# massquantity/tdfo

Hardware: AMD Instinct MI355X
Metric: examples/sec (whole node) DLRM on Criteo-1TB-shaped synthetic (higher is better)
Workload: dtype bf16; 1 GPU; model=DLRM, global_batch=8192, parallelism=single-gpu, tables=criteo-1tb, embedding_dim=128, per_gpu_batch=8192

## Files before the change

csrc/bindings.cpp:

```cpp
#include <cmath>
#include <cstring>

#include <ATen/ATen.h>
#include <ATen/hip/HIPContext.h>
#include <torch/library.h>

#include "tdfo_kernels.h"

namespace {

using at::Tensor;

hipStream_t cur_stream() { return at::hip::getCurrentHIPStream().stream(); }

const uint16_t* bf16_ptr(const Tensor& t) {
  TORCH_CHECK(t.scalar_type() == at::kBFloat16, "expected bf16 tensor");
  return reinterpret_cast<const uint16_t*>(t.data_ptr());
}
uint16_t* bf16_mut(const Tensor& t) {
  TORCH_CHECK(t.scalar_type() == at::kBFloat16, "expected bf16 tensor");
  return reinterpret_cast<uint16_t*>(t.data_ptr());
}
void check_dev(const Tensor& t, const char* name) {
  TORCH_CHECK(t.is_cuda(), name, " must be a GPU tensor");
}
void check_2d_rowmajor(const Tensor& t, const char* name) {
  TORCH_CHECK(t.dim() == 2, name, " must be 2-D");
  TORCH_CHECK(t.stride(1) == 1, name, " must have unit inner stride");
}
bool aligned16(const void* p) { return (reinterpret_cast<uintptr_t>(p) & 15) == 0; }

struct GemmBatch {
  bool on = false;
  std::vector<tdfo::GemmArgs> args;
  std::vector<Tensor> keep;
};
thread_local GemmBatch g_gemm_batch;

void gemm_batch_begin() {
  TORCH_CHECK(!g_gemm_batch.on, "gemm_batch: already open");
  g_gemm_batch.on = true;
}

void gemm_batch_end() {
  GemmBatch& b = g_gemm_batch;
  b.on = false;
  if (!b.args.empty()) tdfo::gemm_group(b.args.data(), (int)b.args.size(), cur_stream());
  b.args.clear();
  b.keep.clear();
}

void gemm(const Tensor& a_in, bool a_col, const Tensor& b_in, bool b_col,
          const c10::optional<Tensor>& bias, bool relu,
          const c10::optional<Tensor>& mask, const c10::optional<Tensor>& out,
          const c10::optional<Tensor>& out32, int64_t splits, const c10::optional<Tensor>& mul,
          const c10::optional<Tensor>& add, const c10::optional<Tensor>& out2, int64_t ldc32,
          int64_t csum_col) {
  check_dev(a_in, "a"); check_dev(b_in, "b");
  check_2d_rowmajor(a_in, "a"); check_2d_rowmajor(b_in, "b");
  const int64_t Ka = a_col ? a_in.size(0) : a_in.size(1);
  const int64_t Kb = b_col ? b_in.size(0) : b_in.size(1);
  TORCH_CHECK(Ka == Kb && Ka > 0, "gemm: K mismatch ", Ka, " vs ", Kb);
  Tensor a = a_in, b = b_in;
  if (Ka % 64) {
    const int64_t Kp = (Ka + 63) / 64 * 64;
    auto pad = [&](const Tensor& t, bool col) {
      Tensor z = col ? at::zeros({Kp, t.size(1)}, t.options()) : at::zeros({t.size(0), Kp}, t.options());
      if (col) z.narrow(0, 0, Ka).copy_(t); else z.narrow(1, 0, Ka).copy_(t);
      return z;
    };
    a = pad(a_in, a_col);
    b = pad(b_in, b_col);
  }
  const int64_t M = a_col ? a.size(1) : a.size(0);
  const int64_t K = a_col ? a.size(0) : a.size(1);
  const int64_t N = b_col ? b.size(1) : b.size(0);
  TORCH_CHECK(M > 0 && N > 0, "gemm: empty output");
  TORCH_CHECK(a.stride(0) % 8 == 0 && b.stride(0) % 8 == 0, "gemm: ld must be multiple of 8");
  TORCH_CHECK(aligned16(a.data_ptr()) && aligned16(b.data_ptr()), "gemm: operands must be 16-B aligned");
  if (a_col) TORCH_CHECK(M % 8 == 0 && M >= 8, "gemm: col-layout A needs M % 8 == 0");
  if (b_col) TORCH_CHECK(N % 8 == 0 && N >= 8, "gemm: col-layout B needs N % 8 == 0");
  TORCH_CHECK(splits >= 1 && splits <= K / 64, "gemm: bad split count");
  TORCH_CHECK(splits == 1 || !(bias || relu || mask),
              "gemm: splits > 1 takes no bias, relu or mask (the epilogue would act on every "
              "partial sum)");
  tdfo::GemmArgs g{};
  g.A = bf16_ptr(a); g.lda = a.stride(0); g.a_col = a_col;
  g.B = bf16_ptr(b); g.ldb = b.stride(0); g.b_col = b_col;
  g.M = (int)M; g.N = (int)N; g.K = (int)K; g.splits = (int)splits;
  if (bias) {
    check_dev(*bias, "bias");
    TORCH_CHECK(bias->scalar_type() == at::kFloat && bias->dim() == 1 && bias->numel() == N,
                "gemm: bias must be fp32 [N] (any stride)");
    g.bias = bias->data_ptr<float>(); g.bias_stride = bias->stride(0);
  }
  g.relu = relu;
  if (mask) {
    check_2d_rowmajor(*mask, "mask");
    TORCH_CHECK(mask->size(0) == M && mask->size(1) == N, "gemm: mask shape");
    g.mask = bf16_ptr(*mask); g.ldm = mask->stride(0);
  }
  TORCH_CHECK(out || out32 || out2, "gemm: need an output");
  if (out) {
    check_2d_rowmajor(*out, "out");
    TORCH_CHECK(out->size(0) == M && out->size(1) == N, "gemm: out shape");
    g.C = bf16_mut(*out); g.ldc = out->stride(0);
    TORCH_CHECK(splits == 1, "gemm: bf16 output requires splits == 1");
  }
  if (out32) {
    TORCH_CHECK(out32->scalar_type() == at::kFloat && out32->is_contiguous(), "gemm: out32 fp32 contiguous");
    const int64_t ld32 = ldc32 > 0 ? ldc32 : N;
    TORCH_CHECK(ld32 >= N && ld32 % 4 == 0, "gemm: ldc32 must be >= N and a multiple of 4");
    TORCH_CHECK(out32->numel() >= splits * M * ld32, "gemm: out32 too small");
    g.C32 = out32->data_ptr<float>(); g.ldc32 = ld32;
    if (csum_col >= 0) {
      TORCH_CHECK(a_col && csum_col >= N && csum_col < ld32,
                  "gemm: csum_col needs a col-layout A and N <= csum_col < ldc32");
      g.csum_on = 1; g.csum_col = (int)csum_col;
    }
  }
  TORCH_CHECK(csum_col < 0 || out32, "gemm: csum_col needs out32");
  auto check_mn = [&](const c10::optional<Tensor>& t, const char* name) {
    check_2d_rowmajor(*t, name);
    TORCH_CHECK(t->size(0) == M && t->size(1) == N && t->stride(0) % 8 == 0 &&
                aligned16(t->data_ptr()), "gemm: ", name, " must be [M, N], 16-B aligned rows");
  };
  if (mul) { check_mn(mul, "mul"); g.mul = bf16_ptr(*mul); g.ldmul = mul->stride(0); }
  if (add) { check_mn(add, "add"); g.add = bf16_ptr(*add); g.ldadd = add->stride(0); }
  if (out2) {
    check_mn(out2, "out2");
    TORCH_CHECK(splits == 1, "gemm: out2 requires splits == 1");
    g.C2 = bf16_mut(*out2); g.ldc2 = out2->stride(0);
  }
  TORCH_CHECK(!(mul || add) || out2, "gemm: mul/add need out2");
  if (g_gemm_batch.on) {
    g_gemm_batch.args.push_back(g);
    g_gemm_batch.keep.push_back(a);
    g_gemm_batch.keep.push_back(b);
    return;
  }
  tdfo::gemm_bf16(g, cur_stream());
}

tdfo::SlotMap make_slots(at::IntArrayRef off, at::IntArrayRef stride, int64_t F) {
  TORCH_CHECK((int64_t)off.size() >= F && (int64_t)stride.size() >= F, "slot map too short");
  tdfo::SlotMap m{};
  for (int64_t i = 0; i < F && i < 32; ++i) { m.off[i] = off[i]; m.stride[i] = stride[i]; }
  return m;
}

void check_inter(int64_t F, int64_t D) {
  TORCH_CHECK(F >= 2 && F <= 32, "interaction: F must be in [2, 32]");
  TORCH_CHECK(D == 16 || D == 32 || D == 64 || D == 128 || D == 256,
              "interaction: D must be 16/32/64/128/256");
}

void check_slots_fit(const Tensor& emb, const tdfo::SlotMap& m, int64_t F, int64_t D, int64_t B) {
  for (int64_t i = 1; i < F; ++i) {
    TORCH_CHECK(m.off[i] % 8 == 0 && m.stride[i] % 8 == 0, "slot offsets must be multiples of 8");
    TORCH_CHECK(m.off[i] >= 0 && m.off[i] + (B - 1) * m.stride[i] + D <= emb.numel(),
                "interaction: slot ", i, " out of range");
  }
}

void interaction_fwd(const Tensor& dense, const Tensor& emb, at::IntArrayRef off,
                     at::IntArrayRef stride, int64_t F, int64_t D, const Tensor& out,
                     int64_t ones_col) {
  check_dev(dense, "dense"); check_dev(emb, "emb"); check_dev(out, "out");
  check_inter(F, D); check_2d_rowmajor(dense, "dense"); check_2d_rowmajor(out, "out");
  const int64_t B = dense.size(0);
  TORCH_CHECK(dense.size(1) >= D && dense.stride(0) % 8 == 0, "dense shape");
  TORCH_CHECK(out.size(0) == B && out.size(1) >= D + F * (F - 1) / 2 && out.size(1) % 8 == 0 &&
              out.stride(0) == out.size(1), "interaction out must be [B, ldo] contiguous, ldo%8==0");
  TORCH_CHECK(emb.is_contiguous() && aligned16(emb.data_ptr()) && aligned16(dense.data_ptr()) &&
              aligned16(out.data_ptr()), "alignment");
  auto m = make_slots(off, stride, F);
  check_slots_fit(emb, m, F, D, B);
  tdfo::interaction_fwd(bf16_ptr(dense), dense.stride(0), bf16_ptr(emb), m, (int)F, (int)D,
                        (int)B, bf16_mut(out), out.stride(0), (int)ones_col, cur_stream());
}

void interaction_bwd(const Tensor& dz, const Tensor& dense, const Tensor& emb,
                     at::IntArrayRef off, at::IntArrayRef stride, int64_t F, int64_t D,
                     const Tensor& d_dense, const Tensor& d_emb, at::IntArrayRef doff,
                     at::IntArrayRef dstride, bool relu_mask) {
  check_dev(dz, "dz"); check_dev(dense, "dense"); check_dev(emb, "emb");
  check_dev(d_dense, "d_dense"); check_dev(d_emb, "d_emb");
  check_inter(F, D);
  check_2d_rowmajor(dz, "dz"); check_2d_rowmajor(dense, "dense"); check_2d_rowmajor(d_dense, "d_dense");
  const int64_t B = dense.size(0);
  TORCH_CHECK(dz.size(0) == B && dz.size(1) >= D + F * (F - 1) / 2, "dz shape");
  TORCH_CHECK(d_dense.size(0) == B && d_dense.size(1) >= D, "d_dense shape");
  TORCH_CHECK(dz.stride(0) % 8 == 0 && aligned16(dz.data_ptr()), "dz alignment");
  TORCH_CHECK(d_dense.stride(0) % 8 == 0 && aligned16(d_dense.data_ptr()) &&
              aligned16(d_emb.data_ptr()), "d_dense / d_emb alignment (16-B row stores)");
  TORCH_CHECK(emb.is_contiguous() && d_emb.is_contiguous(), "emb contiguous");
  auto m = make_slots(off, stride, F);
  auto dm = make_slots(doff, dstride, F);
  check_slots_fit(emb, m, F, D, B);
  check_slots_fit(d_emb, dm, F, D, B);
  tdfo::interaction_bwd(bf16_ptr(dz), dz.stride(0), bf16_ptr(dense), dense.stride(0),
                        bf16_ptr(emb), m, (int)F, (int)D, (int)B, bf16_mut(d_dense),
                        d_dense.stride(0), bf16_mut(d_emb), dm, relu_mask, cur_stream());
}

tdfo::AttnArgs attn_args(const Tensor& qkv, const Tensor& ids, int64_t H, double rate,
                         int64_t seed, const c10::optional<Tensor>& step, int64_t pad_id,
                         bool stream = false) {
  check_dev(qkv, "qkv"); check_dev(ids, "ids");
  TORCH_CHECK(qkv.scalar_type() == at::kFloat && qkv.is_contiguous() && qkv.dim() == 3,
              "attention: qkv fp32 contiguous [B, T, 3E]");
  TORCH_CHECK(ids.scalar_type() == at::kLong && ids.is_contiguous() && ids.dim() == 2 &&
              ids.size(0) == qkv.size(0) && ids.size(1) == qkv.size(1), "attention: ids int64 [B, T]");
  const int64_t E3 = qkv.size(2);
  TORCH_CHECK(E3 % 3 == 0 && H > 0 && (E3 / 3) % H == 0, "attention: 3E must split into H heads");
  if (stream) {
    TORCH_CHECK(qkv.size(1) > tdfo::ATTN_SHORT_MAXT && qkv.size(1) <= tdfo::ATTN_STREAM_MAXT,
                "attention (streaming): 64 < T <= 4096");
  } else {
    TORCH_CHECK(qkv.size(1) <= tdfo::ATTN_LONG_MAXT,
                "attention: T <= 512 (one-wave kernel up to 64, tiled kernel with lse above)");
  }
  TORCH_CHECK(rate >= 0.0 && rate < 1.0, "attention: dropout rate in [0, 1)");
  tdfo::AttnArgs a{};
  a.qkv = qkv.data_ptr<float>(); a.ids = ids.data_ptr<int64_t>();
  a.B = (int)qkv.size(0); a.T = (int)qkv.size(1); a.H = (int)H; a.dk = (int)(E3 / 3 / H);
  a.scale = 1.f / std::sqrt((float)a.dk); a.rate = (float)rate; a.seed = seed; a.pad_id = pad_id;
  if (step) {
    check_dev(*step, "step");
    TORCH_CHECK(step->scalar_type() == at::kLong && step->numel() >= 1, "attention: step int64");
    a.step = step->data_ptr<int64_t>();
  }
  return a;
}

// ... 1970 lines not shown
```

csrc/include/tdfo_kernels.h:

```cpp
#pragma once
#include <hip/hip_runtime.h>
#include <stdint.h>

namespace tdfo {

struct GemmArgs {
  const uint16_t* A; int64_t lda; int a_col;
  const uint16_t* B; int64_t ldb; int b_col;
  int M, N, K, splits;
  const float* bias; int64_t bias_stride;
  int relu;
  const uint16_t* mask; int64_t ldm;
  uint16_t* C; int64_t ldc;
  float* C32; int64_t ldc32;
  const uint16_t* mul; int64_t ldmul;
  const uint16_t* add; int64_t ldadd;
  uint16_t* C2; int64_t ldc2;
  int csum_on, csum_col;
};
void gemm_bf16(const GemmArgs& a, hipStream_t s);


void gemm_group(const GemmArgs* a, int n, hipStream_t s);
int gemm_pairing(int v);
int gemm_policy(int p);

struct SlotMap { int64_t off[32]; int64_t stride[32]; };
void interaction_fwd(const uint16_t* dense, int64_t ld_dense,
                     const uint16_t* emb, const SlotMap& slots, int F, int D,
                     int B, uint16_t* out, int64_t ldo, int ones_col, hipStream_t s);
void interaction_bwd(const uint16_t* dz, int64_t ldz, const uint16_t* dense,
                     int64_t ld_dense, const uint16_t* emb,
                     const SlotMap& slots, int F, int D, int B,
                     uint16_t* d_dense, int64_t ld_ddense, uint16_t* d_emb,
                     const SlotMap& dslots, int relu_mask, hipStream_t s);

void concat_features(const uint16_t* dense, int64_t ld_dense, const uint16_t* emb,
                     const SlotMap& slots, int F, int D, int B, uint16_t* out,
                     hipStream_t s);
void split_features(const uint16_t* dx, int64_t ld_dx, int F, int D, int B,
                    const uint16_t* dense, int64_t ld_dense, uint16_t* d_dense,
                    int64_t ld_ddense, uint16_t* d_emb, const SlotMap& dslots, int relu_mask,
                    hipStream_t s);
void cross_bwd(const uint16_t* dout, const uint16_t* x0, const uint16_t* y, int64_t n,
               uint16_t* dy, uint16_t* dx0, int accumulate, int add_dout, hipStream_t s);

size_t radix_sort_workspace(int64_t n);
int radix_sort_max_bits(int b);
int radix_sort_passes(int key_bits, int64_t n);
int radix_sort_tiled(int v);
int radix_sort_sep_hist(int v);
int radix_sort_pairs_u32(uint32_t* ka, int32_t* va, uint32_t* kb, int32_t* vb, int64_t n,
                         int key_bits, void* ws, hipStream_t s);
int radix_sort_pairs_u64(uint64_t* ka, int32_t* va, uint64_t* kb, int32_t* vb, int64_t n,
                         int key_bits, void* ws, hipStream_t s);

struct BumpArgs {
  void* p[8];
  int is_i64[8];
  int n;
};

struct EmbFwdArgs {
  const float* W; int D;
  int w_bf16 = 0;
  const int64_t* row_offset;
  const int64_t* indices;
  const int64_t* offsets;
  const int64_t* out_off;
  const float* psw;
  int T, B, mean;
  int64_t out_stride;
  void* out; int out_bf16;
  int onehot;
  BumpArgs bumps{};
};
void embedding_bag_fwd(const EmbFwdArgs& a, hipStream_t s);

enum EmbOpt { EMB_SGD = 0, EMB_ROWWISE_ADAGRAD = 1, EMB_ADAM = 2,
              EMB_ADAGRAD = 3, EMB_DENSE_GRAD = 4 };
struct HeadBumps { float* p[4]; int n; };

constexpr int TT_NPARAM = 2400;
constexpr int TT_PART_LD = 2432;
struct TwoTowerArgs {
  const float* X; int64_t ldx;
  const float* P;
  const float* labels; float inv_n;
  const float* loss_scale;
  int half;
  int B;
  float* logits;
  float* dX; int64_t lddx;
  float* part;
  HeadBumps bumps{};
  const float* emb_w = nullptr; const int64_t* ids = nullptr; const int64_t* row_off = nullptr;
};

constexpr int REDUCE_ADAM_MAX_NB = 512;
struct ReduceAdamArgs {
  const float* part; int nparts; int n; int ld;
  float* grad; float* p; float* m; float* v;
  const float* hyper; float beta1, beta2, eps, wd; int adamw;
  double* loss_acc;
  const float* logits = nullptr; const float* labels = nullptr; int nlog = 0; int nb = 0;
  unsigned long long* hist = nullptr;
};

struct EmbBwdArgs {
  float* W; int D;
  const int64_t* row_offset; const int64_t* indices; const int64_t* offsets;
  const int64_t* grad_off;
  const float* psw;
  int T, B, mean; int64_t nnz; int key_bits;
  const void* grad; int grad_bf16; int64_t grad_stride;
  int opt;
  float* state1; float* state2;
  const float* hyper;
  int hyper_n;
  float eps, beta1, beta2, weight_decay;
  float* dense_grad;
  void* workspace; size_t workspace_bytes;
  int segsort;
  int goff_sorted;
  const int32_t* bag_len;
  ReduceAdamArgs side{};
  int side_on = 0;
  TwoTowerArgs tower{};
  int tower_on = 0;
  int side_block0 = 0;
  int w_bf16 = 0;
  int sr = 0;
  uint32_t sr_seed = 0;
  int64_t* sr_counter = nullptr;
};
size_t embedding_bwd_workspace(int64_t nnz, int D);
int embedding_segsort(int v);
void embedding_bwd_fused(const EmbBwdArgs& a, hipStream_t s);
void embedding_bwd_prepare(const EmbBwdArgs& a, hipStream_t s);
void embedding_bwd_apply(const EmbBwdArgs& a, hipStream_t s);

void embedding_dense_update(const EmbBwdArgs& a, int64_t rows, const float* grad, float* clear,
                            hipStream_t s);

struct SynthArgs {
  uint64_t seed; int rank; int64_t batch_index;
  int B, num_dense, T;
  const int64_t* rows; const int* pooling; const int64_t* base;
  int dist; double alpha;
  const float* w_dense; const float* table_bias;
  float* dense; int64_t* ids; float* label;
  const float* index_ptr; uint16_t* x0; int64_t ldx;
};
void synth_criteo(const SynthArgs& a, hipStream_t s);
void synth_ids(const SynthArgs& a, hipStream_t s);
void synth_dense(const SynthArgs& a, hipStream_t s);

struct BotMlpArgs {
  const uint16_t* x; int64_t ldx;
  const uint16_t* w0; const uint16_t* w1; const uint16_t* w2;
  int64_t ldw0, ldw1, ldw2;
  const float* b0; const float* b1; const float* b2;
  int64_t bs0, bs1, bs2;
  uint16_t* y0; uint16_t* y1; uint16_t* y2;
  int64_t ldy0, ldy1, ldy2;
  int M;
  const float* dense = nullptr; int64_t ld_dense = 0; int nd = 0;
  uint16_t* x_out = nullptr;
  const float* label_src = nullptr; float* label_dst = nullptr;
};
bool bottom_mlp_fwd_supported(int k0, int n0, int n1, int n2);
void bottom_mlp_fwd(const BotMlpArgs& a, hipStream_t s);

struct RwBucketArgs {
  const int64_t* ids; const int64_t* meta;
  int nrw, W, B; int64_t cap; int64_t n;
  int64_t* send; int32_t* overflow; int32_t* need;
};
// ... 244 lines not shown
```

csrc/kernels/gemm.hip:

```cpp
#include <cstdlib>

#include "tdfo_common.h"
#include "tdfo_kernels.h"
#include "tdfo_reduce_adam.h"

namespace tdfo {
namespace {

constexpr int BM = 128, BN = 128, BK = 64;
constexpr int TILE_BYTES = BM * BK * 2;
constexpr int STAGE_BYTES = 2 * TILE_BYTES;
constexpr int SMEM_BYTES = 2 * STAGE_BYTES;

typedef __attribute__((address_space(1))) const void* gptr_t;

__device__ __forceinline__ void glds16(const void* src, TDFO_LDS char* dst) {
  __builtin_amdgcn_global_load_lds((gptr_t)src, (TDFO_LDS void*)dst, 16, 0, 0);
}

__device__ __forceinline__ int swz_col(int k) {
  return ((k & 3) | (((k >> 3) & 1) << 2)) << 1;
}

__device__ __forceinline__ void glds_row(const uint16_t* g, int64_t ld, int row0, int rows,
// ... 979 lines not shown
    for (int j = 0; j < 4; ++j) acc[i][j] = (f32x4_t){0.f, 0.f, 0.f, 0.f};

  auto stage = [&](int slot, int kt) {
    TDFO_LDS char* st = smem + slot * P8_STAGE;
    const int k0 = (kt0 + kt) * BK;
#pragma unroll
    for (int u = 0; u < PPW; ++u) {
      const int ii = w * PPW + u, img = ii >> 4;
      if (img < 2)
        glds_piece_asm<A_COL>(p.A, p.lda, m0 + img * 128, p.M, k0, st + img * TILE_BYTES, ii & 15,
                              lane);
      else
        glds_piece_asm<B_COL>(p.B, p.ldb, n0, p.N, k0, st + 2 * TILE_BYTES, ii & 15, lane);
    }
  };
  bf16x8_t af[4], bfr[4];
  auto rd_a = [&](int slot, int half) {
    const TDFO_LDS char* img = smem + slot * P8_STAGE + (ar >> 7) * TILE_BYTES;
#pragma unroll
    for (int i = 0; i < 4; ++i)
      af[i] = A_COL ? frag_col(img, half * 64 + i * 16, grp, lane)
                    : frag_row(img, half * 64 + i * 16, grp, lane);
  };
  auto rd_b = [&](int slot) {
    const TDFO_LDS char* img = smem + slot * P8_STAGE + 2 * TILE_BYTES;
#pragma unroll
    for (int j = 0; j < 4; ++j)
      bfr[j] = B_COL ? frag_col(img, bc + j * 16, grp, lane) : frag_row(img, bc + j * 16, grp, lane);
  };
  auto mm = [&](int half) {
    __builtin_amdgcn_s_setprio(1);
#pragma unroll
    for (int i = 0; i < 4; ++i)
#pragma unroll
      for (int j = 0; j < 4; ++j)
        acc[half * 4 + i][j] =
            __builtin_amdgcn_mfma_f32_16x16x32_bf16(bfr[j], af[i], acc[half * 4 + i][j], 0, 0, 0);
    __builtin_amdgcn_s_setprio(0);
  };
  auto wait_landed = [&](bool one_ahead) {
    if (one_ahead) asm volatile("s_waitcnt vmcnt(%0)" ::"i"(PPW) : "memory");
    else           asm volatile("s_waitcnt vmcnt(0)" ::: "memory");
  };
  if (nk > 0) {
    stage(0, 0);
    if (nk > 1) stage(1, 1);
    wait_landed(nk > 1);
  }
  pp_barrier();
  if (grp == 1) pp_barrier();
  for (int t = 0; t < nk; ++t) {
    const int slot = t % P8_NST;
    const bool ahead = t + 2 < nk;
    rd_b(slot);
    rd_a(slot, 0);
    if (ahead) stage((t + 2) % P8_NST, t + 2);
    asm volatile("s_waitcnt lgkmcnt(0)" ::: "memory");
    pp_barrier();
    mm(0);
    pp_barrier();
    rd_a(slot, 1);
    asm volatile("s_waitcnt lgkmcnt(0)" ::: "memory");
    if (grp == 1 && t + 1 < nk) wait_landed(ahead);
    pp_barrier();
    mm(1);
    if (grp == 0 && t + 1 < nk) wait_landed(ahead);
    pp_barrier();
  }
  if (grp == 0) pp_barrier();
  __syncthreads();
  f32x4_t* red = (f32x4_t*)smem_raw;
  if (grp == 1) {
#pragma unroll
    for (int i = 0; i < 8; ++i)
#pragma unroll
      for (int j = 0; j < 4; ++j) red[(q * 32 + i * 4 + j) * 64 + lane] = acc[i][j];
  }
  __syncthreads();
  if (grp == 1) return;
#pragma unroll
  for (int i = 0; i < 8; ++i)
#pragma unroll
    for (int j = 0; j < 4; ++j) acc[i][j] += red[(q * 32 + i * 4 + j) * 64 + lane];
  pp_epilogue<8, 4>(p, acc, m0 + ar, n0 + bc, lane, ti.split);
}

template <bool A_COL, bool B_COL>
__global__ __launch_bounds__(512, 1) void gemm_p8_kernel(GemmArgs p) {
  extern __shared__ __attribute__((aligned(16))) char smem_raw[];
  gemm_p8_body<A_COL, B_COL>(p, blockIdx.x, smem_raw);
}

template <bool AC0, bool BC0, bool AC1, bool BC1>
__global__ __launch_bounds__(512, 1) void gemm_p8_pair_kernel(GemmArgs p0, GemmArgs p1, int nb0) {
  extern __shared__ __attribute__((aligned(16))) char smem_raw[];
  if ((int)blockIdx.x < nb0) gemm_p8_body<AC0, BC0>(p0, blockIdx.x, smem_raw);
  else                       gemm_p8_body<AC1, BC1>(p1, blockIdx.x - nb0, smem_raw);
}

template <bool A_COL, bool B_COL>
__global__ __launch_bounds__(512, 2) void gemm_pp_kernel(GemmArgs p) {
  extern __shared__ __attribute__((aligned(16))) char smem_raw[];
  gemm_pp_body<128, 2, 128, A_COL, B_COL>(p, blockIdx.x, smem_raw);
}

template <bool AC0, bool BC0, bool AC1, bool BC1>
__global__ __launch_bounds__(512, 2) void gemm_pp_pair_kernel(GemmArgs p0, GemmArgs p1, int nb0,
                                                              int nb01, HeadReduceJob hr) {
  extern __shared__ __attribute__((aligned(16))) char smem_raw[];
  if ((int)blockIdx.x >= nb01) {
    const int slice = threadIdx.x >> 8;
    head_reduce_unit(hr, ((int)blockIdx.x - nb01) * 2 + slice, threadIdx.x & 255,
                     (float(*)[RA_COLS])smem_raw + slice * RA_PH);
    return;
  }
  if ((int)blockIdx.x < nb0) gemm_pp_body<128, 2, 128, AC0, BC0>(p0, blockIdx.x, smem_raw);
  else                       gemm_pp_body<128, 2, 128, AC1, BC1>(p1, blockIdx.x - nb0, smem_raw);
}

int pp_grid(const GemmArgs& a) {
  return ((a.M + 127) / 128) * ((a.N + 127) / 128) * a.splits;
}

template <bool AC, bool BC>
void pp_launch(const GemmArgs& a, hipStream_t s) {
  static bool attr = false;
  if (!attr) {
    TDFO_CHECK_HIP(hipFuncSetAttribute((const void*)gemm_pp_kernel<AC, BC>,
                                       hipFuncAttributeMaxDynamicSharedMemorySize, PPG::LDS));
    attr = true;
  }
  hipLaunchKernelGGL((gemm_pp_kernel<AC, BC>), dim3(pp_grid(a)), dim3(512), PPG::LDS, s, a);
  TDFO_CHECK_HIP(hipGetLastError());
}

template <bool AC0, bool BC0, bool AC1, bool BC1>
void pp_pair_launch(const GemmArgs& a0, const GemmArgs& a1, hipStream_t s) {
  auto fn = gemm_pp_pair_kernel<AC0, BC0, AC1, BC1>;
  static bool attr = false;
  if (!attr) {
    TDFO_CHECK_HIP(hipFuncSetAttribute((const void*)fn, hipFuncAttributeMaxDynamicSharedMemorySize,
                                       PPG::LDS));
    attr = true;
  }
  const int g0 = pp_grid(a0), g01 = g0 + pp_grid(a1);
  HeadReduceJob hr{};
  const int side = head_reduce_take(&hr) ? (head_reduce_units(hr) + 1) / 2 : 0;
  hipLaunchKernelGGL(fn, dim3(g01 + side), dim3(512), PPG::LDS, s, a0, a1, g0, g01, hr);
  TDFO_CHECK_HIP(hipGetLastError());
}

int g_policy = 0;

enum Kern { K_SMALL64 = 64, K_SMALL128 = 128, K_DEEP = 2, K_PP = 3, K_BIG = 4, K_P8 = 8 };

template <bool AC, bool BC>
int choose(const GemmArgs& a) {
  const int t128 = ((a.M + BM - 1) / BM) * ((a.N + BN - 1) / BN) * a.splits;
  const int ktps = (a.K / BK + a.splits - 1) / a.splits;
  const bool big_ok = !a.csum_on && a.K % BK == 0;
  switch (g_policy) {
    case 1: return (!AC && t128 < 256) ? K_SMALL64 : K_SMALL128;
    case 2: return K_DEEP;
    case 3: return K_PP;
    case 4: return big_ok ? K_BIG : K_PP;
    case 8: return big_ok ? K_P8 : K_PP;
    default: break;
  }
  if (g_policy == 5) {
    const int t256 = ((a.M + LBM - 1) / LBM) * ((a.N + BN - 1) / BN) * a.splits;
    if (!AC && t256 < 256 && t128 <= 512 && ktps >= 16) return K_DEEP;
    if (big_ok) return K_BIG;
  } else {
    if (!AC && ktps >= 32 && t128 <= 512) return K_DEEP;
    if (big_ok && t128 >= 1024) return K_BIG;
  }
  if (AC || BC || t128 >= 256) return K_PP;
  return K_SMALL64;
}

template <bool AC, bool BC>
void launch(const GemmArgs& a, int k, hipStream_t s) {
  static bool attr = false;
  if (!attr) {
    TDFO_CHECK_HIP(hipFuncSetAttribute((const void*)gemm_kernel<128, AC, BC>,
                                       hipFuncAttributeMaxDynamicSharedMemorySize, SMEM_BYTES));
    TDFO_CHECK_HIP(hipFuncSetAttribute((const void*)gemm_deep_kernel<AC, BC>,
                                       hipFuncAttributeMaxDynamicSharedMemorySize, DSMEM));
    TDFO_CHECK_HIP(hipFuncSetAttribute((const void*)gemm_big_kernel<AC, BC>,
                                       hipFuncAttributeMaxDynamicSharedMemorySize, LSMEM));
    TDFO_CHECK_HIP(hipFuncSetAttribute((const void*)gemm_p8_kernel<AC, BC>,
                                       hipFuncAttributeMaxDynamicSharedMemorySize, P8_LDS));
    attr = true;
  }
  const int tn = (a.N + BN - 1) / BN;
  switch (k) {
    case K_PP:
      pp_launch<AC, BC>(a, s);
      return;
    case K_BIG:
      hipLaunchKernelGGL((gemm_big_kernel<AC, BC>), dim3(((a.M + LBM - 1) / LBM) * tn * a.splits),
                         dim3(512), LSMEM, s, a);
      break;
    case K_P8:
      hipLaunchKernelGGL((gemm_p8_kernel<AC, BC>), dim3(((a.M + LBM - 1) / LBM) * tn * a.splits),
                         dim3(512), P8_LDS, s, a);
      break;
    case K_DEEP:
      hipLaunchKernelGGL((gemm_deep_kernel<AC, BC>), dim3(((a.M + BM - 1) / BM) * tn * a.splits),
                         dim3(256), DSMEM, s, a);
      break;
    case K_SMALL64:
      if constexpr (!AC) {
        hipLaunchKernelGGL((gemm_kernel<64, AC, BC>), dim3(((a.M + 63) / 64) * tn * a.splits),
                           dim3(256), 2 * (64 * BK * 2 + TILE_BYTES), s, a);
        break;
      }
      [[fallthrough]];
    default:
      hipLaunchKernelGGL((gemm_kernel<128, AC, BC>), dim3(((a.M + BM - 1) / BM) * tn * a.splits),
                         dim3(256), SMEM_BYTES, s, a);
      break;
  }
  TDFO_CHECK_HIP(hipGetLastError());
}

int kernel_of(const GemmArgs& a) {
  if (a.a_col) return a.b_col ? choose<true, true>(a) : choose<true, false>(a);
  return a.b_col ? choose<false, true>(a) : choose<false, false>(a);
}

void launch_any(const GemmArgs& a, hipStream_t s) {
  const int k = kernel_of(a);
  if (a.a_col) {
    if (a.b_col) launch<true, true>(a, k, s); else launch<true, false>(a, k, s);
  } else {
    if (a.b_col) launch<false, true>(a, k, s); else launch<false, false>(a, k, s);
  }
}

int layout_of(const GemmArgs& a) { return (a.a_col ? 2 : 0) | (a.b_col ? 1 : 0); }

int big_grid(const GemmArgs& a) {
  return ((a.M + LBM - 1) / LBM) * ((a.N + BN - 1) / BN) * a.splits;
}

template <bool AC0, bool BC0, bool AC1, bool BC1>
void big_pair_launch(const GemmArgs& a0, const GemmArgs& a1, hipStream_t s) {
  auto fn = gemm_big_pair_kernel<AC0, BC0, AC1, BC1>;
  static bool attr = false;
  if (!attr) {
    TDFO_CHECK_HIP(hipFuncSetAttribute((const void*)fn, hipFuncAttributeMaxDynamicSharedMemorySize,
                                       LSMEM));
    attr = true;
  }
  const int g0 = big_grid(a0);
  hipLaunchKernelGGL(fn, dim3(g0 + big_grid(a1)), dim3(512), LSMEM, s, a0, a1, g0);
  TDFO_CHECK_HIP(hipGetLastError());
}

template <bool AC0, bool BC0, bool AC1, bool BC1>
void p8_pair_launch(const GemmArgs& a0, const GemmArgs& a1, hipStream_t s) {
  auto fn = gemm_p8_pair_kernel<AC0, BC0, AC1, BC1>;
  static bool attr = false;
  if (!attr) {
    TDFO_CHECK_HIP(hipFuncSetAttribute((const void*)fn, hipFuncAttributeMaxDynamicSharedMemorySize,
                                       P8_LDS));
    attr = true;
  }
  const int g0 = big_grid(a0);
  hipLaunchKernelGGL(fn, dim3(g0 + big_grid(a1)), dim3(512), P8_LDS, s, a0, a1, g0);
  TDFO_CHECK_HIP(hipGetLastError());
}

bool try_pair(const GemmArgs& a0, const GemmArgs& a1, hipStream_t s) {
  const int k0 = kernel_of(a0), k1 = kernel_of(a1);
  const int l0 = layout_of(a0), l1 = layout_of(a1);
  if (k0 == K_P8 && k1 == K_P8) {
    if (l0 == 3 && l1 == 1) { p8_pair_launch<true, true, false, true>(a0, a1, s); return true; }
    if (l1 == 3 && l0 == 1) { p8_pair_launch<true, true, false, true>(a1, a0, s); return true; }
    if (l0 == 3 && l1 == 3) { p8_pair_launch<true, true, true, true>(a0, a1, s); return true; }
    return false;
  }
  const bool b0 = k0 == K_BIG || (k1 == K_BIG && k0 == K_DEEP && !a0.csum_on);
  const bool b1 = k1 == K_BIG || (k0 == K_BIG && k1 == K_DEEP && !a1.csum_on);
  if (b0 && b1) {
    if (l0 == 3 && l1 == 1) { big_pair_launch<true, true, false, true>(a0, a1, s); return true; }
    if (l1 == 3 && l0 == 1) { big_pair_launch<true, true, false, true>(a1, a0, s); return true; }
    if (l0 == 3 && l1 == 3) { big_pair_launch<true, true, true, true>(a0, a1, s); return true; }
    return false;
  }
  if (k0 != K_PP || k1 != K_PP) return false;
  if (l0 == 3 && l1 == 1) { pp_pair_launch<true, true, false, true>(a0, a1, s); return true; }
  if (l1 == 3 && l0 == 1) { pp_pair_launch<true, true, false, true>(a1, a0, s); return true; }
  if (l0 == 3 && l1 == 3) { pp_pair_launch<true, true, true, true>(a0, a1, s); return true; }
  return false;
}

int g_pair = 1;

}

int gemm_policy(int p) {
  const int old = g_policy;
  if (p >= 0) g_policy = p;
  return old;
}

void gemm_bf16(const GemmArgs& a, hipStream_t s) { launch_any(a, s); }

int gemm_pairing(int v) {
  const int old = g_pair;
  if (v >= 0) g_pair = v ? 1 : 0;
  return old;
}

void gemm_group(const GemmArgs* a, int n, hipStream_t s) {
  for (int i = 0; i < n;) {
    if (g_pair && i + 1 < n && try_pair(a[i], a[i + 1], s)) {
      i += 2;
      continue;
    }
    gemm_bf16(a[i], s);
    ++i;
  }
}

}
```

tdfo_amd/models/dlrm.py:

```python
from __future__ import annotations

import math
import os
import warnings
from dataclasses import dataclass, field
from typing import List, Optional, Sequence

import torch

from ..utils.capture import graph_capture
from .. import ops
from .dlrm_dcn import DCNMixin
from .dlrm_streams import StreamGraphsMixin
from .dlrm_multirank import MultiRankStreamsMixin
from ..parallel.comm import as_comm, dense_comm_for
from ..sparse.planner import ShardingPlan, plan_sharding
from ..sparse.sharded import ShardedEmbeddingBags
from ..sparse.tables import EmbOptimConfig, TableConfig
from ..utils.flat import FlatParams

CRITEO_1TB_ROWS = [39884406, 39043, 17289, 7420, 20263, 3, 7120, 1543, 63, 38532951, 2953546,
                   403346, 10, 2208, 11938, 155, 4, 976, 14, 39979771, 25641295, 39664984, 585935,
                   12972, 108, 36]
CRITEO_KAGGLE_ROWS = [1460, 583, 10131227, 2202608, 305, 24, 12517, 633, 3, 93145, 5683, 8351593,
# ... 112 lines not shown
@dataclass
class Lin:
    name: str
    in_real: int
    in_k: int
    out: int
    bcol: int
    wcols: int

    @property
    def bias_in_k(self) -> bool:
        return self.bcol < self.in_k


WCOL_PAD = 64


def make_lin(name: str, in_real: int, out: int) -> Lin:
    in_k = pad64(in_real)
    if in_real < in_k:
        return Lin(name, in_real, in_k, out, in_real, in_k)
    return Lin(name, in_real, in_k, out, in_k, in_k + WCOL_PAD)




class DLRMTrainer(StreamGraphsMixin, MultiRankStreamsMixin, DCNMixin):

    def __init__(self, cfg: DLRMConfig, batch_size: int, device, group=None, rank: int = 0,
                 world_size: int = 1, plan: Optional[ShardingPlan] = None):
        self.cfg = cfg
        if cfg.dense_comm not in ("fp32", "bf16"):
            raise ValueError(f"dense_comm must be fp32 or bf16, got {cfg.dense_comm!r}")
        if cfg.opt_placement not in (None, "one_pass", "split_main"):
            raise ValueError(f"opt_placement must be one_pass or split_main, "
                             f"got {cfg.opt_placement!r}")
        if cfg.opt_placement is None:
            cfg.opt_placement = "split_main" if cfg.interaction == "dcn" else "one_pass"
        self.B = B = int(batch_size)
        self.device = dev = torch.device(device)
        self.group = group
        self.comm = as_comm(group) if world_size > 1 else None
        self.dcomm = dense_comm_for(self.comm) if world_size > 1 else None
        self.rank = rank
        self.world = world_size
        D = cfg.embedding_dim
        T = cfg.num_tables
        self.F = F = T + 1
        assert cfg.bottom[-1] == D, "bottom MLP must end at the embedding dim"
        assert cfg.top[-1] == 1
        assert cfg.interaction != "dcn" or cfg.dcn_rank % 64 == 0, "dcn_rank must be a multiple of 64"
        torch.manual_seed(cfg.seed)
        optim = EmbOptimConfig(cfg.emb_opt, lr=cfg.emb_lr, eps=cfg.emb_eps)
        tables = cfg.tables()
        self.plan = plan or plan_sharding(tables, world_size, optim, batch_per_rank=B,
                                          pooling=cfg.pooling_factors(), strategy=cfg.sharding,
                                          dp_rule=cfg.dp_rule, table_dtype=cfg.table_dtype)
        self.emb = ShardedEmbeddingBags(tables, self.plan, rank, B, cfg.pooling_factors(), dev,
                                        optim, group=self.comm, seed=cfg.seed,
                                        rw_capacity=cfg.rw_capacity, rw_comm=cfg.rw_comm,
                                        rw_exchange=cfg.rw_exchange, table_dtype=cfg.table_dtype)
        if self.dcomm is not None:
            self.emb.dp_comm = self.dcomm
        fp = FlatParams()
        dims = [cfg.num_dense] + cfg.bottom
        self.bottom_layers = [make_lin(f"bot{i}", a, b)
                              for i, (a, b) in enumerate(zip(dims[:-1], dims[1:]))]
        if cfg.interaction == "dot":
            self.top_real = D + F * (F - 1) // 2
        else:
            self.top_real = F * D
        tdims = [self.top_real] + cfg.top[:-1]
        self.top_layers = [make_lin(f"top{i}", a, b)
                           for i, (a, b) in enumerate(zip(tdims[:-1], tdims[1:]))]
        for L in self.bottom_layers + self.top_layers:
            fp.add(L.name + ".w", (L.out, L.wcols))
        self.dcn_u = []
        if cfg.interaction == "dcn":
            Wd = self.top_real
            for i in range(cfg.dcn_layers):
                fp.add(f"dcn{i}.v", (cfg.dcn_rank, Wd))
                u = make_lin(f"dcn{i}.u", cfg.dcn_rank, Wd)
                self.dcn_u.append(u)
                fp.add(u.name + ".w", (u.out, u.wcols))
        self.head_k = tdims[-1]
        fp.add("head", (self.head_k + 1,))
        opt = DENSE_OPTS[cfg.dense_opt]
        self.dense_opt = opt
        fp.finalize(dev, with_adam=opt in (ops.OPT_ADAMW, ops.OPT_ADAM))
        self.fp = fp
        self._ar_split = fp.offset(self.top_layers[0].name + ".w")
        self._init_dense()
        if world_size > 1:
            self.comm.broadcast(fp.p, src=0)
        fp.sync_bf16()
        self._defer_top_wgrad = (world_size > 1 if cfg.defer_wgrad is None
                                 else bool(cfg.defer_wgrad))
        bf = torch.bfloat16

        def z(*shape, dt=bf):
            return torch.zeros(*shape, dtype=dt, device=dev)

        def act_in(L: Lin):
            t = z(B, L.wcols)
            t[:, L.bcol] = 1.0
            return t

        self.x0 = act_in(self.bottom_layers[0])
        self.bot_in = [self.x0] + [act_in(L) for L in self.bottom_layers[1:]]
        self.h_out = z(B, D)
        Lb = self.bottom_layers
        self._fused_bottom = (
            dev.type == "cuda" and len(Lb) == 3 and D == Lb[2].out
            and os.environ.get("TDFO_FUSED_BOTTOM", "1") != "0"
            and Lb[0].in_k == Lb[0].wcols and not Lb[1].bias_in_k and not Lb[2].bias_in_k
            and Lb[1].in_k == Lb[0].out and Lb[2].in_k == Lb[1].out
            and ops.bottom_mlp_fwd_ok(Lb[0].in_k, Lb[0].out, Lb[1].out, Lb[2].out))
        self._bot_load_fold = os.environ.get("TDFO_BOT_LOAD_FOLD", "1") != "0"
        self._head_side = os.environ.get("TDFO_HEAD_SIDE", "1") != "0"
        self.bot_grad = [z(B, L.out) for L in self.bottom_layers]
        self.top_in = [act_in(L) for L in self.top_layers]
        self.t_out = z(B, self.head_k)
        self.top_grad = [z(B, L.out) for L in self.top_layers]
        self.dz = z(B, self.top_layers[0].in_k)
        self.label = z(B, dt=torch.float32)
        self.ids = torch.zeros(self.emb.nnz_local, dtype=torch.int64, device=dev)
        self.emb.bind_ids(self.ids)
        if cfg.interaction == "dcn":
            Lc, Wd, r = cfg.dcn_layers, self.top_real, cfg.dcn_rank
            self.dcn_x = [z(B, Wd) for _ in range(Lc)] + [self.top_in[0]]
            self.dcn_h = [act_in(u) for u in self.dcn_u]
            self.dcn_y = [z(B, Wd) for _ in range(Lc)]
            self.dcn_dx = [z(B, Wd) for _ in range(Lc + 1)]
            self.dcn_dx0acc = z(B, Wd)
            nb = Lc if self._defer_top_wgrad else 1
            self.dcn_dhl = [z(B, r) for _ in range(nb)]
            self.dcn_dyl = [z(B, Wd) for _ in range(nb)]
        self._x0_alias = False
        if (cfg.interaction == "dcn" and not self._defer_top_wgrad
                and self.emb.alias_pooled(self.dcn_x[0], self.dcn_dx[0], D)):
            self._x0_alias = True
            self.h_out = self.dcn_x[0][:, :D]
        self.logits = z(B, dt=torch.float32)
        self.nparts = ops.head_parts(B)
        self.head_part = z(self.nparts * (self.head_k + 2), dt=torch.float32)
        self.loss_sum = z(1, dt=torch.float32)
        self._pair_bwd = dev.type == "cuda"
        dcn = cfg.interaction == "dcn"
        if dev.type == "cuda" and not os.environ.get("TDFO_GEMM_POLICY"):
            ops.gemm_policy(5 if dcn else 0)
        self._gemm_pol = ops.gemm_policy(-1) if dev.type == "cuda" else None
        self._csum = not (dcn and dev.type == "cuda" and ops.gemm_policy(-1) in (4, 5))
        self._wg_slots = (128 if self._pair_bwd else 256) if not self._csum else 0
        self.wslab = {}
        self._slab_sums = []
        self._segments = []
        self._opt_sums_slabs = dev.type == "cuda" and world_size == 1
        max_slab = 1
        if cfg.interaction == "dcn":
            max_slab = self._wg_splits(cfg.dcn_rank, self.top_real) * cfg.dcn_rank * self.top_real
        self.slab = z(max_slab, dt=torch.float32)
        for L in self.bottom_layers + self.top_layers + self.dcn_u:
            S = self._wg_splits(L.out, self._wgrad_n(L))
            if S > 1:
                sl = z(S * L.out * L.wcols, dt=torch.float32)
                self.wslab[L.name] = (sl, S)
                if self._opt_sums_slabs:
                    self._segments.append((fp.offset(L.name + ".w"), sl, S))
                else:
                    self._slab_sums.append((fp.offset(L.name + ".w"), sl, S,
                                            fp.grad(L.name + ".w").view(-1)))
        if cfg.interaction == "dcn" and dev.type == "cuda":
            for i in range(cfg.dcn_layers):
                S = self._wg_splits(cfg.dcn_rank, self.top_real)
                if S > 1:
                    sl = z(S * cfg.dcn_rank * self.top_real, dt=torch.float32)
                    self.wslab[f"dcn{i}.v"] = (sl, S)
                    if self._opt_sums_slabs:
                        self._segments.append((fp.offset(f"dcn{i}.v"), sl, S))
                    else:
                        self._slab_sums.append((fp.offset(f"dcn{i}.v"), sl, S,
                                                fp.grad(f"dcn{i}.v").view(-1)))
        self.dense_hyper = torch.tensor([cfg.dense_lr, 0.0, 1.0], dtype=torch.float32, device=dev)
        self.emb_hyper = torch.tensor([cfg.emb_lr, 0.0], dtype=torch.float32, device=dev)
        self.slot_off = [0] + list(self.emb.slot_off)
        self.slot_stride = [0] + list(self.emb.slot_stride)
        self.graph = None
        self.steps = 0
        self._ps = torch.cuda.Stream(device=dev) if dev.type == "cuda" else None
        self.pipeline = bool(cfg.pipeline) and world_size > 1
        self._pipe_lookup = self.pipeline and bool(cfg.pipeline_lookup)
        self._rw_lagged = self.pipeline and bool(self.emb.rw_tables) and self.emb.rw_dynamic
        on_cuda = dev.type == "cuda"
        self._ev_loaded = torch.cuda.Event() if (on_cuda and self._pipe_lookup) else None
        self._ev_lookup = torch.cuda.Event() if (on_cuda and self._pipe_lookup) else None
        self._next = None
        self._primed = False
        self._mstream = False
        self._bstg = None
        self._ms = None
        self._whole_capture = False
        self._cap_origin = None
        self._stg = None
        self._mr = None
        self._graph_layout = 0
        self._insrc = None
        self._src_copy_stream = None
        self._src_copy_owner = None

    def weight(self, name: str):
        L = next(L for L in self.bottom_layers + self.top_layers + self.dcn_u if L.name == name)
        W = self.fp.param(name + ".w")
        return W[:, :L.in_real], W[:, L.bcol]

    def _init_dense(self):
        g = torch.Generator(device="cpu")
        g.manual_seed(self.cfg.seed + 7)
        fp = self.fp
        for L in self.bottom_layers + self.top_layers + self.dcn_u:
            W = fp.param(L.name + ".w")
            W.zero_()
            w = torch.randn(L.out, L.in_real, generator=g) * math.sqrt(2.0 / (L.in_real + L.out))
            W[:, :L.in_real] = w.to(W.device)
            if not L.name.startswith("dcn"):
                W[:, L.bcol] = (torch.randn(L.out, generator=g) * math.sqrt(1.0 / L.out)).to(W.device)
        if self.cfg.interaction == "dcn":
            r, w = self.cfg.dcn_rank, self.top_real
            for i in range(self.cfg.dcn_layers):
                fp.param(f"dcn{i}.v").copy_(torch.randn(r, w, generator=g) * math.sqrt(2.0 / (r + w)))
        K = self.head_k
        h = fp.param("head")
        h[:K] = (torch.randn(K, generator=g) * math.sqrt(2.0 / (K + 1))).to(h.device)
        h[K] = 0.0

    def load_batch(self, dense: torch.Tensor, ids: torch.Tensor, label: torch.Tensor,
                   on_device: bool = False):
        if self.graph == "streams":
            stg = self._bstg
            if self._ms_load_ids(ids, on_device, dense, label):
                if stg is None:
                    ops.batch_load(dense, self.x0, ids[:0], self.ids[:0], label, self.label)
                elif not on_device:
                    stg[0].copy_(dense, non_blocking=True)
                    stg[1].copy_(label.reshape(-1), non_blocking=True)
                return
            if stg is not None:
                stg[0].copy_(dense, non_blocking=True)
                stg[1].copy_(label.reshape(-1), non_blocking=True)
                self.ids.copy_(ids)
                return
        ops.batch_load(dense, self.x0, ids, self.ids, label, self.label)

    def set_copy_stream(self, stream, owner=None):
        if self.graph is not None:
            raise RuntimeError("set the copy stream before capture_graph()")
        self._src_copy_stream = stream
        self._src_copy_owner = owner

    def attach_in_step_source(self, src):
        if self.world != 1 or self.pipeline:
            raise ValueError("in-step batch generation is for the one-GPU step")
        if self.graph is not None:
            raise RuntimeError("attach the in-step source before capture_graph()")
        self._insrc = src
        src.bind(self.dense_hyper[1:2])

    def _s_gen_ids(self):
        if self._insrc is not None:
            self._insrc.gen_ids(self.ids)

    def _s_gen_dense(self):
        if self._insrc is not None:
            self._insrc.gen_dense(self.x0, self.label)

    def prime(self, dense: torch.Tensor, ids: torch.Tensor, label: torch.Tensor):
        assert self.pipeline, "prime() needs DLRMConfig(pipeline=True) and world_size > 1"
        self.load_batch(dense, ids, label)
        self.emb._rw_lag_pending = False
        if not self.emb.fwd_prep_noop:
            self.emb.stage_fwd_prep(self.ids)
        self.emb.stage_fwd_ids_exchange(async_op=True)
        if self._pipe_lookup:
            self.emb.ids_exchange_wait()
            self.emb.stage_fwd_lookup()
            self._m_out_exchange_next()
        self._next = (dense, ids, label)
        self._primed = True
        self._mr_inflight = True

    def set_next_batch(self, dense: torch.Tensor, ids: torch.Tensor, label: torch.Tensor):
        if self.graph == "mstreams":
            self._mr_stage_next(dense, ids, label)
            return
        self._next = (dense, ids, label)

    def _m_load_next(self):
        if self._whole_capture:
            sx, si, sl = self._stg
            self.x0.copy_(sx)
            self.ids.copy_(si)
            self.label.copy_(sl)
            return
        dense, ids, label = self._next
        ops.batch_load(dense, self.x0, ids, self.ids, label, self.label)

    def _m_ids_exchange_next(self):
        self.emb.stage_fwd_ids_exchange(async_op=True, lagged=self._rw_lagged)

    def _rw_resolve(self):
        if self._rw_lagged and self.emb.rw_resolve_need():
            self.sync_streams()
            self.emb.rw_redo()

    def _fwd(self, L: Lin, x, out, relu=True):
        W = self.fp.bf16(L.name + ".w")
        bias = None if L.bias_in_k else self.fp.param(L.name + ".w")[:, L.bcol]
        ops.gemm(x[:, :L.in_k], False, W[:, :L.in_k], False, bias, relu, None, out, None, 1)

    def _bwd(self, L: Lin, x, dy, dx, x_is_relu, wgrad_now: bool = True):
        if not wgrad_now:
            self._dgrad(L, x, dy, dx, x_is_relu)
            return
        with ops.gemm_batch(self._pair_bwd and dx is not None):
            self._wgrad_gemm(L, x, dy)
            self._dgrad(L, x, dy, dx, x_is_relu)

    def _wg_splits(self, M: int, N: int) -> int:
        return ops.wgrad_splits(M, N, self.B, 256, slots=self._wg_slots)

    def _wgrad_n(self, L: Lin) -> int:
        return L.in_k if self._csum else L.wcols

    def _wgrad(self, L: Lin, x, dy):
        self._wgrad_gemm(L, x, dy)

    def _wgrad_gemm(self, L: Lin, x, dy):
        csum = -1 if (L.bias_in_k or not self._csum) else L.bcol
        n = self._wgrad_n(L)
        g = self.fp.grad(L.name + ".w").view(-1)
        if L.name in self.wslab:
            sl, S = self.wslab[L.name]
            ops.gemm(dy, True, x[:, :n], True, None, False, None, None, sl, S,
                     ldc32=L.wcols, csum_col=csum)
        else:
            ops.gemm(dy, True, x[:, :n], True, None, False, None, None, g, 1,
                     ldc32=L.wcols, csum_col=csum)
        return None

    def _dgrad(self, L: Lin, x, dy, dx, x_is_relu):
        if dx is not None:
            n = min(dx.shape[1], L.in_k)
            W = self.fp.bf16(L.name + ".w")
            ops.gemm(dy, False, W[:, :n], True, None, False,
                     x[:, :n] if x_is_relu else None, dx[:, :n], None, 1)

    def _stages(self):
        emb = self.emb
        top_wgrad = [("c", self._s_top_wgrad)] if self._defer_top_wgrad else []
        prep = [] if emb.fwd_prep_noop else [("c", lambda: emb.stage_fwd_prep(self.ids))]
        if self.pipeline:
            eprep = [("e", k[1]) for k in prep]
            if self._pipe_lookup:
                return [
                    ("c", self._s_bottom_fwd),
                    ("m", self._m_fwd_wait),
                    ("c", self._s_top),
                    ("m", emb.backward_start),
                ] + top_wgrad + [
                    ("m", self._m_allreduce_top_start),
                    ("c", self._s_bottom_bwd),
                    ("m", self._m_allreduce_start),
                    ("m", emb.backward_wait),
                    ("e", self._s_emb_update),
                    ("em", self._m_load_next),
                    ("em", self._m_mark_loaded),
                ] + eprep + [
                    ("em", self._m_ids_exchange_next),
                    ("em", emb.ids_exchange_wait),
                    ("e", emb.stage_fwd_lookup),
                    ("em", self._m_out_exchange_next),
                    ("m", self._m_allreduce_wait),
                    ("c", self._s_dense_update),
                    ("jw", None),
                ]
            return [
                ("m", emb.ids_exchange_wait),
                ("c", emb.stage_fwd_lookup),
                ("m", emb.stage_fwd_out_exchange),
                ("c", self._s_bottom_fwd),
                ("m", self._m_fwd_wait),
                ("c", self._s_top),
                ("m", emb.backward_start),
            ] + top_wgrad + [
                ("m", self._m_allreduce_top_start),
                ("c", self._s_bottom_bwd),
                ("m", self._m_allreduce_start),
                ("m", emb.backward_wait),
                ("e", self._s_emb_update),
                ("em", self._m_load_next),
            ] + eprep + [
                ("em", self._m_ids_exchange_next),
                ("m", self._m_allreduce_wait),
                ("c", self._s_dense_update),
                ("j", None),
            ]
        gen = [("c", lambda: (self._s_gen_ids(), self._s_gen_dense()))] if self._insrc else []
        return gen + prep + [
            ("m", emb.stage_fwd_ids_exchange),
            ("c", emb.stage_fwd_lookup),
            ("m", emb.stage_fwd_out_exchange),
            ("c", self._s_bottom_fwd),
            ("m", self._m_fwd_wait),
            ("c", self._s_top),
            ("m", emb.backward_start),
        ] + top_wgrad + [
            ("m", self._m_allreduce_top_start),
            ("c", self._s_bottom_bwd),
            ("m", self._m_allreduce_start),
            ("m", emb.backward_wait),
            ("e", self._s_emb_update),
            ("m", self._m_allreduce_wait),
            ("c", self._s_dense_update),
            ("j", None),
        ]

    def _wait(self, dst, src):
        o = self._cap_origin
        if o is None or dst == o or src == o:
            dst.wait_stream(src)
        else:
            o.wait_stream(src)
            dst.wait_stream(o)

    def _side(self):
        if self.device.type != "cuda" or self.world == 1:
            return None
        if getattr(self, "_sides", None) is None:
            self._sides = torch.cuda.Stream(device=self.device)
        return self._sides

    def _run_stage(self, kind, fn, graph=None):
        se = self._side()
        if kind == "j":
            if se is not None:
                self._wait(torch.cuda.current_stream(), se)
            self._on_side = False
            return
        if kind == "jw":
            if se is not None and self._ev_loaded is not None:
                torch.cuda.current_stream().wait_event(self._ev_loaded)
            self._on_side = False
            return
        if kind in ("e", "em") and se is not None:
            if not getattr(self, "_on_side", False):
                self._wait(se, torch.cuda.current_stream())
                self._on_side = True
            with torch.cuda.stream(se):
                graph.replay() if graph is not None else fn()
            return
        graph.replay() if graph is not None else fn()

    def _forward_backward(self):
        self._on_side = False
        for kind, fn in self._stages():
            self._run_stage(kind, fn)

    def _s_bottom_fwd(self, staged=None):
        if self._fused_bottom:
            Ls = self.bottom_layers
            bias = [None if L.bias_in_k else self.fp.param(L.name + ".w")[:, L.bcol] for L in Ls]
            ops.bottom_mlp_fwd(self.bot_in[0], self.fp.bf16(Ls[0].name + ".w"),
                               self.fp.bf16(Ls[1].name + ".w"), self.fp.bf16(Ls[2].name + ".w"),
                               bias[0], bias[1], bias[2], self.bot_in[1], self.bot_in[2],
                               self.h_out, dense=None if staged is None else staged[0],
                               label=None if staged is None else (staged[1], self.label))
            return
        n = len(self.bottom_layers)
        for i, L in enumerate(self.bottom_layers):
            out = self.bot_in[i + 1][:, :L.out] if i + 1 < n else self.h_out
            self._fwd(L, self.bot_in[i], out)

    def _m_fwd_wait(self):
        if self._whole_capture:
# ... 352 lines not shown
```

Measured before the change: 20.30 million examples/s.

## Add skinny-N MFMA weight-gradient kernel for narrow-input layers

Adds a dedicated split-K MFMA kernel for weight-gradient GEMMs whose output width N is at most 16, such as the first bottom-MLP layer with only a few dense inputs. It also narrows the wgrad N to the live columns for those layers. The goal is to avoid launching 128-wide tiles that are mostly padding and to spread K across more blocks. In exchange, split counts can exceed the old limit, and more validation paths now route through the new kernel.

```diff
diff --git a/csrc/bindings.cpp b/csrc/bindings.cpp
--- a/csrc/bindings.cpp
+++ b/csrc/bindings.cpp
@@ -79,8 +79,19 @@
   TORCH_CHECK(a.stride(0) % 8 == 0 && b.stride(0) % 8 == 0, "gemm: ld must be multiple of 8");
   TORCH_CHECK(aligned16(a.data_ptr()) && aligned16(b.data_ptr()), "gemm: operands must be 16-B aligned");
   if (a_col) TORCH_CHECK(M % 8 == 0 && M >= 8, "gemm: col-layout A needs M % 8 == 0");
-  if (b_col) TORCH_CHECK(N % 8 == 0 && N >= 8, "gemm: col-layout B needs N % 8 == 0");
-  TORCH_CHECK(splits >= 1 && splits <= K / 64, "gemm: bad split count");
+  bool skinny = false;
+  if (a_col && b_col && out32 && out32->scalar_type() == at::kFloat && !out && !out2 && !bias &&
+      !relu && !mask && !mul && !add && csum_col < 0 && splits >= 1) {
+    tdfo::GemmArgs q{};
+    q.A = bf16_ptr(a); q.lda = a.stride(0); q.a_col = 1;
+    q.B = bf16_ptr(b); q.ldb = b.stride(0); q.b_col = 1;
+    q.M = (int)M; q.N = (int)N; q.K = (int)K; q.splits = (int)splits;
+    q.C32 = out32->data_ptr<float>(); q.ldc32 = ldc32 > 0 ? ldc32 : N;
+    skinny = tdfo::gemm_takes_skinny(q);
+  }
+  if (b_col && !skinny) TORCH_CHECK(N % 8 == 0 && N >= 8, "gemm: col-layout B needs N % 8 == 0");
+  TORCH_CHECK(splits >= 1 && (splits <= K / 64 || (skinny && splits <= 1024)),
+              "gemm: bad split count");
   TORCH_CHECK(splits == 1 || !(bias || relu || mask),
               "gemm: splits > 1 takes no bias, relu or mask (the epilogue would act on every "
               "partial sum)");
diff --git a/csrc/include/tdfo_kernels.h b/csrc/include/tdfo_kernels.h
--- a/csrc/include/tdfo_kernels.h
+++ b/csrc/include/tdfo_kernels.h
@@ -24,6 +24,9 @@
 void gemm_group(const GemmArgs* a, int n, hipStream_t s);
 int gemm_pairing(int v);
 int gemm_policy(int p);
+bool wgrad_skinny_ok(const GemmArgs& a);
+void wgrad_skinny(const GemmArgs& a, hipStream_t s);
+bool gemm_takes_skinny(const GemmArgs& a);
 
 struct SlotMap { int64_t off[32]; int64_t stride[32]; };
 void interaction_fwd(const uint16_t* dense, int64_t ld_dense,
diff --git a/csrc/kernels/gemm.hip b/csrc/kernels/gemm.hip
--- a/csrc/kernels/gemm.hip
+++ b/csrc/kernels/gemm.hip
@@ -1155,7 +1155,8 @@
 
 int g_policy = 0;
 
-enum Kern { K_SMALL64 = 64, K_SMALL128 = 128, K_DEEP = 2, K_PP = 3, K_BIG = 4, K_P8 = 8 };
+enum Kern { K_SMALL64 = 64, K_SMALL128 = 128, K_DEEP = 2, K_PP = 3, K_BIG = 4, K_P8 = 8,
+            K_SKINNY = 16 };
 
 template <bool AC, bool BC>
 int choose(const GemmArgs& a) {
@@ -1170,6 +1171,7 @@
     case 8: return big_ok ? K_P8 : K_PP;
     default: break;
   }
+  if (AC && BC && wgrad_skinny_ok(a)) return K_SKINNY;
   if (g_policy == 5) {
     const int t256 = ((a.M + LBM - 1) / LBM) * ((a.N + BN - 1) / BN) * a.splits;
     if (!AC && t256 < 256 && t128 <= 512 && ktps >= 16) return K_DEEP;
@@ -1235,6 +1237,10 @@
 
 void launch_any(const GemmArgs& a, hipStream_t s) {
   const int k = kernel_of(a);
+  if (k == K_SKINNY) {
+    wgrad_skinny(a, s);
+    return;
+  }
   if (a.a_col) {
     if (a.b_col) launch<true, true>(a, k, s); else launch<true, false>(a, k, s);
   } else {
@@ -1312,6 +1318,8 @@
 
 void gemm_bf16(const GemmArgs& a, hipStream_t s) { launch_any(a, s); }
 
+bool gemm_takes_skinny(const GemmArgs& a) { return kernel_of(a) == K_SKINNY; }
+
 int gemm_pairing(int v) {
   const int old = g_pair;
   if (v >= 0) g_pair = v ? 1 : 0;
diff --git a/csrc/kernels/wgrad_skinny.hip b/csrc/kernels/wgrad_skinny.hip
--- /dev/null
+++ b/csrc/kernels/wgrad_skinny.hip
@@ -0,0 +1,115 @@
+#include <cstdlib>
+
+#include "tdfo_common.h"
+#include "tdfo_kernels.h"
+
+namespace tdfo {
+namespace {
+
+constexpr int WS_MB = 32;
+constexpr int WS_BK = 64;
+
+__global__ __launch_bounds__(256) void wgrad_skinny_kernel(GemmArgs p) {
+  __shared__ f32x4_t red[3][2][64];
+  const int tid = threadIdx.x, lane = tid & 63;
+  const int w = __builtin_amdgcn_readfirstlane(tid >> 6);
+  const int i = lane & 15, g = lane >> 4;
+  const int mblocks = (p.M + WS_MB - 1) / WS_MB;
+  const int bid = xcd_remap((int)blockIdx.x, (int)gridDim.x);
+  const int split = bid / mblocks;
+  const int m = (bid - split * mblocks) * WS_MB + 2 * i;
+  const int ktiles = p.K / WS_BK;
+  const int per = (ktiles + p.splits - 1) / p.splits;
+  const int kt0 = split * per;
+  const int nk = max(0, min(ktiles, kt0 + per) - kt0);
+  const bool m_ok = m < p.M;
+  const bool n_ok = i < p.N;
+  const uint16_t* a_ptr = p.A + (m_ok ? m : 0);
+  const uint16_t* b_ptr = p.B + (n_ok ? i : 0);
+
+  f32x4_t acc[2] = {{0.f, 0.f, 0.f, 0.f}, {0.f, 0.f, 0.f, 0.f}};
+  for (int t = w; t < nk; t += 4) {
+    const int64_t k0 = (int64_t)(kt0 + t) * WS_BK + 8 * g;
+    uint32_t a[2][8];
+    uint32_t b[2][8];
+#pragma unroll
+    for (int h = 0; h < 2; ++h)
+#pragma unroll
+      for (int j = 0; j < 8; ++j) {
+        const int64_t k = k0 + 32 * h + j;
+        a[h][j] = *(const uint32_t*)(a_ptr + k * p.lda);
+      }
+#pragma unroll
+    for (int h = 0; h < 2; ++h)
+#pragma unroll
+      for (int j = 0; j < 8; ++j) {
+        const int64_t k = k0 + 32 * h + j;
+        b[h][j] = b_ptr[k * p.ldb];
+      }
+#pragma unroll
+    for (int h = 0; h < 2; ++h) {
+      uint32_t lo[4], hi[4], bb[4];
+#pragma unroll
+      for (int q = 0; q < 4; ++q) {
+        lo[q] = (a[h][2 * q] & 0xffffu) | (a[h][2 * q + 1] << 16);
+        hi[q] = (a[h][2 * q] >> 16) | (a[h][2 * q + 1] & 0xffff0000u);
+        bb[q] = b[h][2 * q] | (b[h][2 * q + 1] << 16);
+      }
+      const bf16x8_t bf = __builtin_bit_cast(bf16x8_t, bb);
+      acc[0] = __builtin_amdgcn_mfma_f32_16x16x32_bf16(bf, __builtin_bit_cast(bf16x8_t, lo),
+                                                       acc[0], 0, 0, 0);
+      acc[1] = __builtin_amdgcn_mfma_f32_16x16x32_bf16(bf, __builtin_bit_cast(bf16x8_t, hi),
+                                                       acc[1], 0, 0, 0);
+    }
+  }
+
+  if (w > 0) {
+    red[w - 1][0][lane] = acc[0];
+    red[w - 1][1][lane] = acc[1];
+  }
+  __syncthreads();
+  if (w > 0) return;
+#pragma unroll
+  for (int v = 0; v < 3; ++v) {
+    acc[0] += red[v][0][lane];
+    acc[1] += red[v][1][lane];
+  }
+  if (!m_ok) return;
+  float* c32 = p.C32 + ((int64_t)split * p.M + m) * p.ldc32 + 4 * g;
+#pragma unroll
+  for (int c = 0; c < 2; ++c) {
+    float* o = c32 + c * p.ldc32;
+    if (4 * g + 4 <= p.N) {
+      *(f32x4_t*)o = acc[c];
+    } else {
+#pragma unroll
+      for (int r = 0; r < 4; ++r)
+        if (4 * g + r < p.N) o[r] = acc[c][r];
+    }
+  }
+}
+
+const bool g_wgrad_skinny = [] {
+  const char* e = getenv("TDFO_WGRAD_SKINNY");
+  return !(e && *e && atoi(e) == 0);
+}();
+
+}
+
+bool wgrad_skinny_ok(const GemmArgs& a) {
+  if (!g_wgrad_skinny) return false;
+  if (!a.a_col || !a.b_col || a.N < 1 || a.N > 16 || a.M < 2 || a.splits < 1) return false;
+  if (!a.C32 || a.C || a.C2 || a.bias || a.relu || a.mask || a.mul || a.add || a.csum_on)
+    return false;
+  if ((a.M & 1) || (a.lda & 1) || ((uintptr_t)a.A & 3)) return false;
+  if ((a.ldc32 & 3) || ((uintptr_t)a.C32 & 15) || a.ldc32 < a.N) return false;
+  return a.K >= WS_BK && a.K % WS_BK == 0;
+}
+
+void wgrad_skinny(const GemmArgs& a, hipStream_t s) {
+  const int grid = a.splits * ((a.M + WS_MB - 1) / WS_MB);
+  hipLaunchKernelGGL(wgrad_skinny_kernel, dim3(grid), dim3(256), 0, s, a);
+  TDFO_CHECK_HIP(hipGetLastError());
+}
+
+}
diff --git a/tdfo_amd/models/dlrm.py b/tdfo_amd/models/dlrm.py
--- a/tdfo_amd/models/dlrm.py
+++ b/tdfo_amd/models/dlrm.py
@@ -288,6 +288,7 @@
         self._gemm_pol = ops.gemm_policy(-1) if dev.type == "cuda" else None
         self._csum = not (dcn and dev.type == "cuda" and ops.gemm_policy(-1) in (4, 5))
         self._wg_slots = (128 if self._pair_bwd else 256) if not self._csum else 0
+        self._skinny_wgrad = dev.type == "cuda" and os.environ.get("TDFO_WGRAD_SKINNY", "1") != "0"
         self.wslab = {}
         self._slab_sums = []
         self._segments = []
@@ -297,7 +298,7 @@
             max_slab = self._wg_splits(cfg.dcn_rank, self.top_real) * cfg.dcn_rank * self.top_real
         self.slab = z(max_slab, dt=torch.float32)
         for L in self.bottom_layers + self.top_layers + self.dcn_u:
-            S = self._wg_splits(L.out, self._wgrad_n(L))
+            S = self._wg_splits(L.out, self._wgrad_tile_n(L))
             if S > 1:
                 sl = z(S * L.out * L.wcols, dt=torch.float32)
                 self.wslab[L.name] = (sl, S)
@@ -465,6 +466,12 @@
         return ops.wgrad_splits(M, N, self.B, 256, slots=self._wg_slots)
 
     def _wgrad_n(self, L: Lin) -> int:
+        live = (L.bcol + 16) // 16 * 16
+        if self._skinny_wgrad and L.bias_in_k and live <= 16:
+            return live
+        return self._wgrad_tile_n(L)
+
+    def _wgrad_tile_n(self, L: Lin) -> int:
         return L.in_k if self._csum else L.wcols
 
     def _wgrad(self, L: Lin, x, dy):
```

Result: no change. 20.24 million examples/s (median of 2 runs) (-0.3%).
